# spdes/chirpgp

Hardware: AMD Instinct MI355X
Metric: filter+smoother trial-steps/s (batch x T / wall) (higher is better)
Workload: dtype f64; 1 GPU; C2: discrete EKF+EKS (demos/ekfs_mle.py model); d=4, T=10000, batch_per_gpu=1000, global_batch=1000, parallelism=trials sharded x1

## Files before the change

### chirpgp_amd/csrc/cgp_walk4.hpp

```cpp
#pragma once
#include <atomic>
#include "cgp_coop8.hpp"

namespace cgp {

constexpr int kWalkRec = 37;
constexpr int kWalkG = 0, kWalkC = 16, kWalkc = 32;
constexpr int kWalkAhead = 2;
static_assert(kWalk4LdsBytes == sizeof(double) * 64 * kWalkRec, "walk4_smoother_ok (cgp_route.hpp) budgets the records of walk4_smoother_kernel");
constexpr int kWalkMapDoubles = 40;
struct Walk4Operands { double g, C, c; };

CGP_DEV double blk_bcast0(double x) {
    return dpp_banks_f64<kRowRor12, 0x8>(dpp_banks_f64<kRowRor8, 0x4>(dpp_banks_f64<kRowRor4, 0x2>(x, x), x), x);
}

template <class Elem, int MODE = kWalkWhole, bool SEL = false>
__global__ void __launch_bounds__(64) walk4_smoother_kernel(SmootherIO io, ModelArgs ma) {
    static_assert(Elem::D == 4, "d = 4 kernel");
    static_assert(!(SEL && MODE == kWalkCompose), "pass 1 of the time-split form writes nothing");
    __shared__ double recs[64 * kWalkRec];
    __shared__ double selbuf[SEL ? 128 : 1];
    __shared__ double ghrule[SEL ? 2 * kGhMaxOrder : 1];
    const int lane = threadIdx.x;
    const int r = lane >> 4, b = (lane >> 2) & 3, q = lane & 3;
    const int64_t trial = (MODE == kWalkWhole) ? (int64_t)blockIdx.x : (int64_t)(blockIdx.x / (unsigned)io.segs);
    const int seg = (MODE == kWalkWhole) ? 0 : (int)(blockIdx.x % (unsigned)io.segs);
    if (trial >= io.B) return;

    Elem elem;
    elem.setup(ma, trial);
    if constexpr (SEL) { sel_stage_rule(io.sel, ghrule, lane); wave_lds_fence(); }
    if constexpr (Elem::USES_SIGMA) elem.sg.stage(dyn_lds(), lane, 64, 4);
    const int64_t T = io.T;
    const double* __restrict__ mfs = io.mfs + trial * T * 4;
    const double* __restrict__ Pfs = io.Pfs + trial * T * 16;
    double* __restrict__ mss = io.mss + trial * T * 4;
    double* __restrict__ Pss = io.Pss + trial * T * 16;
    OobWindow wPs, wms;
    wPs.init((MODE == kWalkCompose || !io.Pss) ? nullptr : Pss, T * 128); wms.init((MODE == kWalkCompose || !io.mss) ? nullptr : mss, T * 32);
    const int64_t hi_first = (MODE == kWalkWhole) ? T - 2 : T - 2 - 64 * (int64_t)seg * io.tiles_per_seg;
    const int64_t hi_stop = (MODE == kWalkWhole) ? 0 : max((int64_t)0, hi_first - 64 * (int64_t)io.tiles_per_seg + 1);
    if (hi_first < 0 && MODE != kWalkWhole) return;
    const unsigned offP = (unsigned)b * 128u + (unsigned)(4 * r + q) * 8u;
    const unsigned offm = (q == 0) ? (unsigned)b * 32u + (unsigned)r * 8u : kOobOffset;
    const int oGa = kWalkG + q * 4 + r, oGb = kWalkG + r * 4 + q, oC = kWalkC + r * 4 + q, oc = kWalkc + r;

    double Ps = Pfs[(T - 1) * 16 + ((r >= q) ? r * 4 + q : q * 4 + r)];
    double ms = mfs[(T - 1) * 4 + r];
    double Acc = (r == q) ? 1.0 : 0.0;
    if constexpr (MODE == kWalkCompose) { Ps = 0.0; ms = 0.0; }
    if (MODE != kWalkCompose && seg == 0) {
        if (lane < 16 && (!SEL || io.Pss)) Pss[(T - 1) * 16 + lane] = Pfs[(T - 1) * 16 + lane];
        if (lane < 4 && (!SEL || io.mss)) mss[(T - 1) * 4 + lane] = mfs[(T - 1) * 4 + lane];
        if constexpr (SEL) { if (lane == 0) sel_write(io.sel, ghrule, trial * T + T - 1, mfs[(T - 1) * 4 + io.sel.comp], Pfs[(T - 1) * 16 + io.sel.comp * 5]); }
    }
    const bool sel_var_lane = SEL && r == io.sel.comp && q == io.sel.comp, sel_mean_lane = SEL && r == io.sel.comp && q == 0;
    if constexpr (MODE == kWalkApply) {
        const double* __restrict__ maps = io.ws + trial * io.segs * kWalkMapDoubles;
        for (int s2 = 0; s2 < seg; s2++) {
            const double* __restrict__ mp_ = maps + s2 * kWalkMapDoubles;
            const double gA = mp_[q * 4 + r], Cs = mp_[16 + r * 4 + q], cs = mp_[32 + r];
            const double Wc = mfma4x4(Ps, gA, 0.0);
            ms = mfma4x4(gA, ms, cs);
            Ps = mfma4x4(gA, Wc, Cs);
        }
    }

    auto request = [&](int64_t base, Vec<4>& mf, Sym<4>& Pf) {
        const int64_t t = base + lane;
        load_vec<4>(mfs + (t >= 0 ? t : 0) * 4, mf);
        load_sym<4>(Pfs + (t >= 0 ? t : 0) * 16, Pf);
    };
    auto write_record = [&](bool valid, const Mat<4>& G, const Vec<4>& c, const Sym<4>& C) {
        double* mine = recs + lane * kWalkRec;
        CGP_UNROLL for (int a = 0; a < 4; a++) {
            CGP_UNROLL for (int k = 0; k < 4; k++) {
                mine[kWalkG + a * 4 + k] = valid ? G.a[a][k] : 0.0;
                mine[kWalkC + a * 4 + k] = valid ? C(a, k) : 0.0;
            }
            mine[kWalkc + a] = valid ? c.v[a] : 0.0;
        }
    };
    auto scan = [&]() {
        CGP_UNROLL for (int i = 3; i >= 0; i--) {
            const double* p3 = recs + (16 * i + 4 * b + 3) * kWalkRec;
            double M = p3[oGb], C = p3[oC], c = p3[oc];
            CGP_UNROLL for (int j = 2; j >= 0; j--) {
                double* pj = recs + (16 * i + 4 * b + j) * kWalkRec;
                const double g = pj[oGa], Cj = pj[oC], cj = pj[oc];
                M = mfma4x4(g, M, 0.0);
                c = mfma4x4(g, c, cj);
                const double Tt = mfma4x4(C, g, 0.0);
                C = mfma4x4(Tt, g, Cj);
                pj[oGb] = M; pj[oC] = C; pj[oc] = c;
            }
        }
    };
    auto walk = [&](int64_t base) {
        auto fetch = [&](int Q, Walk4Operands& o) {
            const double* p = recs + ((4 * Q + (MODE == kWalkCompose ? 0 : b)) & 63) * kWalkRec;
            o.g = p[oGa]; o.C = p[oC]; o.c = p[oc];
        };
        Walk4Operands ring[kWalkAhead + 1];
        CGP_UNROLL for (int a = 0; a < kWalkAhead; a++) fetch(15 - a, ring[a]);
        CGP_UNROLL for (int Q = 15; Q >= 0; Q--) {
            fetch(Q - kWalkAhead, ring[(15 - Q + kWalkAhead) % (kWalkAhead + 1)]);
            const Walk4Operands& cur = ring[(15 - Q) % (kWalkAhead + 1)];
            if constexpr (MODE == kWalkCompose) {
                Acc = mfma4x4(cur.g, Acc, 0.0);
                ms = mfma4x4(cur.g, ms, cur.c);
                const double Tt = mfma4x4(Ps, cur.g, 0.0);
                Ps = mfma4x4(cur.g, Tt, cur.C);
            } else {
                const double W = mfma4x4(Ps, cur.g, 0.0);
                const double msn = mfma4x4(cur.g, ms, cur.c);
                const double Psn = mfma4x4(cur.g, W, cur.C);
                const unsigned step = (unsigned)(base + 4 * Q);
                wPs.store(Psn, offP + step * 128u);
                wms.store(msn, offm + step * 32u);
                if constexpr (SEL) {
                    if (sel_var_lane) selbuf[64 + 4 * Q + b] = Psn;
                    if (sel_mean_lane) selbuf[4 * Q + b] = msn;
                }
                Ps = blk_bcast0(Psn);
                ms = blk_bcast0(msn);
            }
        }
    };

    Vec<4> mf; Sym<4> Pf;
    if constexpr (Elem::HAS_SPEC) {
        {
            Mat<4> G; Vec<4> c; Sym<4> C;
            request(hi_first - 63, mf, Pf);
            const bool valid = hi_first - 63 + lane >= 0;
            if (valid) elem.map(mf, Pf, G, c, C);
            write_record(valid, G, c, C);
            wave_lds_fence();
            request(hi_first - 127, mf, Pf);
        }
        for (int64_t hi = hi_first; hi >= hi_stop; hi -= 64) {
            const int64_t base = hi - 63;
            Vec<4> mf2; Sym<4> Pf2;
            request(base - 128, mf2, Pf2);
            Mat<4> G; Vec<4> c; Sym<4> C; bool ok;
            elem.map_spec(mf, Pf, G, c, C, ok);
            scan();
            wave_lds_fence();
            walk(base);
            wave_lds_fence();
            if constexpr (SEL) { if (base + lane >= 0) sel_write(io.sel, ghrule, trial * T + base + lane, selbuf[lane], selbuf[64 + lane]); }
            if (__builtin_expect(__builtin_amdgcn_ballot_w64(!ok) != 0, 0)) elem.map(mf, Pf, G, c, C);
            write_record(base - 64 + lane >= 0, G, c, C);
            wave_lds_fence();
            mf = mf2; Pf = Pf2;
        }
    } else {
        request(hi_first - 63, mf, Pf);
        for (int64_t hi = hi_first; hi >= hi_stop; hi -= 64) {
            const int64_t base = hi - 63;
            {
                Mat<4> G; Vec<4> c; Sym<4> C;
                const bool valid = base + lane >= 0;
                if (valid) elem.map(mf, Pf, G, c, C);
                write_record(valid, G, c, C);
            }
            wave_lds_fence();
            request(base - 64, mf, Pf);
            scan();
            wave_lds_fence();
            walk(base);
            wave_lds_fence();
            if constexpr (SEL) { if (base + lane >= 0) sel_write(io.sel, ghrule, trial * T + base + lane, selbuf[lane], selbuf[64 + lane]); }
        }
    }
    if constexpr (MODE == kWalkCompose) {
        double* __restrict__ out = io.ws + (trial * io.segs + seg) * kWalkMapDoubles;
        if (b == 0) {
            out[r * 4 + q] = Acc;
            out[16 + r * 4 + q] = Ps;
            if (q == 0) out[32 + r] = ms;
        }
    }
}

template <class Elem>
inline hipError_t launch_walk4_smoother(const SmootherIO& io, const ModelArgs& ma, hipStream_t stream) {
    if (io.B <= 0 || io.T <= 0) return hipSuccess;
    if (!walk4_smoother_ok(io.T, ma)) return hipErrorInvalidValue;
    return launch_walk_smoother<Elem, walk4_smoother_kernel<Elem, kWalkWhole, false>, walk4_smoother_kernel<Elem, kWalkWhole, true>,
                                walk4_smoother_kernel<Elem, kWalkCompose, false>, walk4_smoother_kernel<Elem, kWalkApply, false>,
                                walk4_smoother_kernel<Elem, kWalkApply, true>>(io, ma, stream, kWalkMapDoubles);
}

}
```

Before: 3.849 billion trial-steps/s.

## Widen smoother scan blocks from four to eight steps to shorten the carry chain

The in-LDS local scan now composes each lane-group's records in chains of eight, running two independent chains interleaved with double-buffered operand fetches, instead of four chains of four. The walk then consumes two quad-steps per iteration from the same carried state and broadcasts that state only once per eight-step block. This halves the serial mfma plus cross-lane broadcast dependency along the time walk and exposes more instruction-level parallelism. The cost is a longer serial chain inside the scan phase and more registers held for the operand ring.

```diff
diff --git a/chirpgp_amd/csrc/cgp_walk4.hpp b/chirpgp_amd/csrc/cgp_walk4.hpp
--- a/chirpgp_amd/csrc/cgp_walk4.hpp
+++ b/chirpgp_amd/csrc/cgp_walk4.hpp
@@ -83,17 +83,24 @@
         }
     };
     auto scan = [&]() {
-        CGP_UNROLL for (int i = 3; i >= 0; i--) {
-            const double* p3 = recs + (16 * i + 4 * b + 3) * kWalkRec;
-            double M = p3[oGb], C = p3[oC], c = p3[oc];
-            CGP_UNROLL for (int j = 2; j >= 0; j--) {
-                double* pj = recs + (16 * i + 4 * b + j) * kWalkRec;
-                const double g = pj[oGa], Cj = pj[oC], cj = pj[oc];
-                M = mfma4x4(g, M, 0.0);
-                c = mfma4x4(g, c, cj);
-                const double Tt = mfma4x4(C, g, 0.0);
-                C = mfma4x4(Tt, g, Cj);
-                pj[oGb] = M; pj[oC] = C; pj[oc] = c;
+        auto rec = [&](int i, int j) { return recs + (32 * i + 8 * b + j) * kWalkRec; };
+        auto fetch = [&](int j, Walk4Operands (&o)[2]) {
+            CGP_UNROLL for (int i = 0; i < 2; i++) { const double* p = rec(i, j); o[i].g = p[oGa]; o[i].C = p[oC]; o[i].c = p[oc]; }
+        };
+        double M[2], C[2], c[2], Tt[2];
+        CGP_UNROLL for (int i = 0; i < 2; i++) { const double* p7 = rec(i, 7); M[i] = p7[oGb]; C[i] = p7[oC]; c[i] = p7[oc]; }
+        Walk4Operands ring[2][2];
+        fetch(6, ring[0]);
+        CGP_UNROLL for (int j = 6; j >= 0; j--) {
+            if (j > 0) fetch(j - 1, ring[(7 - j) & 1]);
+            const Walk4Operands (&o)[2] = ring[(6 - j) & 1];
+            CGP_UNROLL for (int i = 0; i < 2; i++) M[i] = mfma4x4(o[i].g, M[i], 0.0);
+            CGP_UNROLL for (int i = 0; i < 2; i++) Tt[i] = mfma4x4(C[i], o[i].g, 0.0);
+            CGP_UNROLL for (int i = 0; i < 2; i++) c[i] = mfma4x4(o[i].g, c[i], o[i].c);
+            CGP_UNROLL for (int i = 0; i < 2; i++) C[i] = mfma4x4(Tt[i], o[i].g, o[i].C);
+            CGP_UNROLL for (int i = 0; i < 2; i++) {
+                double* pj = rec(i, j);
+                pj[oGb] = M[i]; pj[oC] = C[i]; pj[oc] = c[i];
             }
         }
     };
@@ -102,29 +109,38 @@
             const double* p = recs + ((4 * Q + (MODE == kWalkCompose ? 0 : b)) & 63) * kWalkRec;
             o.g = p[oGa]; o.C = p[oC]; o.c = p[oc];
         };
-        Walk4Operands ring[kWalkAhead + 1];
-        CGP_UNROLL for (int a = 0; a < kWalkAhead; a++) fetch(15 - a, ring[a]);
-        CGP_UNROLL for (int Q = 15; Q >= 0; Q--) {
-            fetch(Q - kWalkAhead, ring[(15 - Q + kWalkAhead) % (kWalkAhead + 1)]);
-            const Walk4Operands& cur = ring[(15 - Q) % (kWalkAhead + 1)];
+        auto apply = [&](int Q, const Walk4Operands& o, double& Psn, double& msn) {
+            const double W = mfma4x4(Ps, o.g, 0.0);
+            msn = mfma4x4(o.g, ms, o.c);
+            Psn = mfma4x4(o.g, W, o.C);
+            const unsigned step = (unsigned)(base + 4 * Q);
+            wPs.store(Psn, offP + step * 128u);
+            wms.store(msn, offm + step * 32u);
+            if constexpr (SEL) {
+                if (sel_var_lane) selbuf[64 + 4 * Q + b] = Psn;
+                if (sel_mean_lane) selbuf[4 * Q + b] = msn;
+            }
+        };
+        Walk4Operands ring[kWalkAhead + 1][2];
+        auto fetch_octad = [&](int O, Walk4Operands (&o)[2]) {
+            fetch(2 * O, o[0]);
+            if constexpr (MODE != kWalkCompose) fetch(2 * O + 1, o[1]);
+        };
+        CGP_UNROLL for (int a = 0; a < kWalkAhead; a++) fetch_octad(7 - a, ring[a]);
+        CGP_UNROLL for (int O = 7; O >= 0; O--) {
+            fetch_octad(O - kWalkAhead, ring[(7 - O + kWalkAhead) % (kWalkAhead + 1)]);
+            const Walk4Operands (&cur)[2] = ring[(7 - O) % (kWalkAhead + 1)];
             if constexpr (MODE == kWalkCompose) {
-                Acc = mfma4x4(cur.g, Acc, 0.0);
-                ms = mfma4x4(cur.g, ms, cur.c);
-                const double Tt = mfma4x4(Ps, cur.g, 0.0);
-                Ps = mfma4x4(cur.g, Tt, cur.C);
+                Acc = mfma4x4(cur[0].g, Acc, 0.0);
+                ms = mfma4x4(cur[0].g, ms, cur[0].c);
+                const double Tt = mfma4x4(Ps, cur[0].g, 0.0);
+                Ps = mfma4x4(cur[0].g, Tt, cur[0].C);
             } else {
-                const double W = mfma4x4(Ps, cur.g, 0.0);
-                const double msn = mfma4x4(cur.g, ms, cur.c);
-                const double Psn = mfma4x4(cur.g, W, cur.C);
-                const unsigned step = (unsigned)(base + 4 * Q);
-                wPs.store(Psn, offP + step * 128u);
-                wms.store(msn, offm + step * 32u);
-                if constexpr (SEL) {
-                    if (sel_var_lane) selbuf[64 + 4 * Q + b] = Psn;
-                    if (sel_mean_lane) selbuf[4 * Q + b] = msn;
-                }
-                Ps = blk_bcast0(Psn);
-                ms = blk_bcast0(msn);
+                double PsHi, msHi, PsLo, msLo;
+                apply(2 * O + 1, cur[1], PsHi, msHi);
+                apply(2 * O, cur[0], PsLo, msLo);
+                Ps = blk_bcast0(PsLo);
+                ms = blk_bcast0(msLo);
             }
         }
     };
```

Result: no change. 3.865 billion trial-steps/s, median of 2 (+0.4%).
